# Unsigned-Long/slam-tricks

Hardware: AMD Instinct MI355X
Metric: LM iterations/sec + residuals/sec, 1k-cam/100k-pt BA (higher is better)
Workload: dtype f64

## Files before the change

include/stba.h:

```cpp
#ifndef STBA_H
#define STBA_H

#include <stddef.h>

#ifdef __cplusplus
extern "C" {
#endif

#define STBA_VERSION 6

enum {
    STBA_OK = 0,
    STBA_ERR_INVALID_ARGUMENT = -1,
    STBA_ERR_NO_DEVICE = -2,
    STBA_ERR_HIP = -3,
    STBA_ERR_NOT_POSITIVE_DEFINITE = -4,
    STBA_ERR_ALLOC = -5,
    STBA_ERR_STATE = -6,
    STBA_ERR_CALLBACK = -7,
    STBA_ERR_NO_SOLUTION = -8
};

const char* stba_status_string(int status);
const char* stba_last_error(void);
// ... 57 lines not shown
int stba_comm_create(stba_comm** out, const char id[STBA_COMM_ID_BYTES], int rank, int world_size, int device);
int stba_comm_destroy(stba_comm* comm);
int stba_comm_rank(const stba_comm* comm, int* rank, int* world_size);
int stba_comm_allreduce_sum(stba_comm* comm, void* buf_dev, size_t count, void* hip_stream);
int stba_comm_allreduce_hook(void* user, void* buf_dev, size_t count, void* hip_stream);

typedef struct stba_ba stba_ba;

int stba_ba_create(stba_ba** out, int n_cams, int n_pts, int n_obs, const double* cams,
                   const double* pts, const int* obs_cam, const int* obs_pt, const double* obs_feat,
                   const unsigned char* cam_fixed, const unsigned char* pt_fixed, void* hip_stream);
int stba_ba_destroy(stba_ba* ba);
enum { STBA_SCHUR_AUTO = 0, STBA_SCHUR_PAIRS = 1, STBA_SCHUR_DENSE = 2 };
int stba_ba_set_schur_mode(stba_ba* ba, int mode);
int stba_ba_schur_mode(const stba_ba* ba, int* mode);
int stba_ba_set_params(stba_ba* ba, const double* cams, const double* pts);
int stba_ba_get_params(stba_ba* ba, double* cams, double* pts);
int stba_ba_set_features(stba_ba* ba, const double* obs_feat);
int stba_get_device(int* device);
int stba_set_device(int device);
typedef int (*stba_ba_linearize_fn)(void* user, const double* cams, const double* pts, double* r, double* Jc, double* Jp);
int stba_ba_set_host_linearizer(stba_ba* ba, stba_ba_linearize_fn fn, void* user);
int stba_ba_set_allreduce(stba_ba* ba, stba_allreduce_fn fn, void* user, int rank, int world_size);
int stba_ba_set_comm(stba_ba* ba, stba_comm* comm);
int stba_ba_reduced_dim(const stba_ba* ba, int* n, int* n_padded);

int stba_ba_evaluate(stba_ba* ba, double* cost, double* r, double* Jc, double* Jp);
int stba_ba_cost(stba_ba* ba, double* cost);
int stba_ba_normal_blocks(stba_ba* ba, double* Hcc, double* gc, double* Hpp, double* gp);
int stba_ba_reduced_system(stba_ba* ba, const double* dc, const double* dp, double* S, double* rhs);
// ... 219 lines not shown
```

slam-tricks_amd/__init__.py:

```python
import ctypes as C
import os
import sys

import numpy as np

_HERE = os.path.dirname(os.path.abspath(__file__))
LIB_PATH = os.environ.get("STBA_LIB") or os.path.join(_HERE, "libstba.so")
TRACE_COLS = 7
TERM_REASON = {0: "none", 1: "gradient", 2: "function", 3: "parameter", 4: "max_iter",
               5: "min_radius", 6: "solver_fail", 7: "fixed", 8: "user"}
_lib = None


class StbaError(RuntimeError):
    def __init__(self, code, where):
        self.code = code
        msg = _lib.stba_last_error().decode() if _lib is not None else ""
        super().__init__(f"{where}: status {code} ({_lib.stba_status_string(code).decode()}) {msg}")


class LMOptions(C.Structure):
    _fields_ = [("max_num_iterations", C.c_int), ("initial_trust_region_radius", C.c_double),
                ("max_trust_region_radius", C.c_double), ("min_trust_region_radius", C.c_double),
                ("min_relative_decrease", C.c_double), ("min_lm_diagonal", C.c_double),
# ... 44 lines not shown
           "stba_ba_create_ex", "stba_ba_set_pcg", "stba_ba_last_pcg_summary", "stba_ba_schur_apply",
           "stba_ba_last_pcg_iterations", "stba_ba_time_schur_apply",
           "stba_ba_set_trust_region", "stba_ba_last_dogleg_summary",
           "stba_ba_set_inner_iterations", "stba_ba_inner_sweep", "stba_ba_last_inner_summary",
           "stba_pg_covariance_default_options", "stba_pg_covariance", "stba_pg_covariance_columns", "stba_pg_gauge_check",
           "stba_pg_set_information", "stba_pg_set_sqrt_information", "stba_pg_has_information",
           "stba_pg_set_loss", "stba_pg_has_loss",
           "stba_pg_set_priors", "stba_pg_prior_count", "stba_pg_evaluate_priors", "stba_pg_prior_kernel_geometry",
           "stba_ba_set_loss", "stba_ba_has_loss", "stba_ba_loss_kernel_geometry",
           "stba_ba_set_information", "stba_ba_set_sqrt_information", "stba_ba_has_information", "stba_ba_get_sqrt_information",
           "stba_ba_set_pose_priors", "stba_ba_pose_prior_count", "stba_ba_evaluate_pose_priors", "stba_ba_pose_prior_kernel_geometry",
           "stba_ba_set_relative_poses", "stba_ba_relative_pose_count", "stba_ba_evaluate_relative_poses",
           "stba_ba_relative_pose_kernel_geometry",
           "stba_ba_set_landmark_priors", "stba_ba_landmark_prior_count", "stba_ba_evaluate_landmark_priors",
           "stba_ba_landmark_prior_kernel_geometry",
           "stba_live_device_buffers"]


def lib():
    global _lib
    if _lib is None:
        if not os.path.exists(LIB_PATH):
            raise ImportError(f"{LIB_PATH} is missing: run `python __graft_entry__.py build` "
                              "(hipcc, gfx950).  There is no CPU fallback.")
        if "torch" not in sys.modules and os.environ.get("STBA_NO_TORCH_PRELOAD", "0") != "1":
            try:
                import torch
            except Exception:
                pass
        L = C.CDLL(LIB_PATH)
# ... 515 lines not shown
    def time_linearize(self, reps=20):
        ms = C.c_double()
        _chk(lib().stba_ba_time_linearize(self._h, int(reps), C.byref(ms)), "stba_ba_time_linearize")
        return ms.value

    SCHUR_AUTO, SCHUR_PAIRS, SCHUR_DENSE = 0, 1, 2

    def set_schur_mode(self, mode):
        _chk(lib().stba_ba_set_schur_mode(self._h, int(mode)), "stba_ba_set_schur_mode")

    def schur_mode(self):
        m = C.c_int()
        _chk(lib().stba_ba_schur_mode(self._h, C.byref(m)), "stba_ba_schur_mode")
        return m.value

    def set_pcg(self, preconditioner="jacobi", eta=0.1, min_iterations=0, max_iterations=500, check_every=4):
        pc = PRECONDITIONERS[preconditioner] if isinstance(preconditioner, str) else int(preconditioner)
        _chk(lib().stba_ba_set_pcg(self._h, pc, C.c_double(eta), int(min_iterations), int(max_iterations), int(check_every)),
             "stba_ba_set_pcg")

    def pcg_summary(self):
        s = PCGSummary()
        _chk(lib().stba_ba_last_pcg_summary(self._h, C.byref(s)), "stba_ba_last_pcg_summary")
        return s

    def pcg_iterations(self, n):
        out = np.zeros(int(n), dtype=np.int32)
        _chk(lib().stba_ba_last_pcg_iterations(self._h, _p(out), int(n)), "stba_ba_last_pcg_iterations")
        return out

# ... 506 lines not shown
```

slam-tricks_amd/build.py:

```python
import os
import subprocess
import sys

HERE = os.path.dirname(os.path.abspath(__file__))
CSRC = os.path.join(HERE, "csrc")
SOURCES = ["dense_chol.hip", "ba_kernels.hip", "stba_engine.hip", "ba_linear.hip", "ba_allreduce.hip", "ba_solve.hip", "ba_stages.hip", "dense_engine.hip", "calib.hip", "ba_factors.hip", "pg_engine.hip", "pg_linearize.hip", "pg_coarse.hip", "pg_pcg.hip", "pg_prior.hip", "small_dense.hip", "two_view.hip", "covariance.hip", "pg_covariance.hip", "iterative_schur.hip", "dogleg.hip", "inner_iterations.hip", "ba_prior.hip", "ba_between.hip", "ba_landmark_prior.hip", "calib_io.cpp", "comm.cpp"]
HEADERS = ["common.hpp", "lm_policy.hpp", "ba_kernels.hpp", "schur_plan.hpp", "chol_schedule.hpp", "small_linalg.hpp", "iterative_schur.hpp", "dogleg.hpp", "dogleg_select.hpp", "inner_iterations.hpp", "inner_policy.hpp", "pg_covariance.hpp", "robust_loss.hpp", "ba_prior.hpp", "ba_between.hpp", "ba_landmark_prior.hpp", "ba_features.hpp", "ba_factor_input.hpp", "ba_engine.hpp", "pg_plan.hpp", "pg_engine.hpp", "pg_device.hpp", "pg_edge.hpp", "inner_plan.hpp", "dd6.hpp", os.path.join("..", "..", "include", "stba.h")]
LIB = os.path.join(HERE, "libstba.so")
FLAGS = ["-O3", "-std=c++17", "--offload-arch=gfx950", "-fPIC", "-munsafe-fp-atomics", "-Wall",
         "-Wno-unused-function", "-Wno-unused-result"]


if os.environ.get("STBA_DEBUG_KNOBS", "0") not in ("", "0"):
    FLAGS.append("-DSTBA_DEBUG_KNOBS")


def _stale():
    if not os.path.exists(LIB):
        return True
    t = os.path.getmtime(LIB)
    deps = [os.path.join(CSRC, s) for s in SOURCES + HEADERS] + [os.path.abspath(__file__)]
    return any(os.path.getmtime(d) > t for d in deps)


# ... 63 lines not shown
```

slam-tricks_amd/csrc/ba_engine.hpp:

```cpp
#pragma once
#include <memory>
#include <vector>

#include "ba_kernels.hpp"
#include "ba_prior.hpp"
#include "ba_between.hpp"
#include "ba_landmark_prior.hpp"
#include "iterative_schur.hpp"
#include "ba_features.hpp"
#include "inner_plan.hpp"

namespace stba {

enum { SC_COST2 = 0, SC_GPMAX0 = 8, SC_MAX_WORLD = 64 };
enum { TS_COST2 = 0, TS_STEP2 = 1, TS_X2 = 2, TS_MODEL = 3, TS_TIMEOUT = 4, TS_CAM = 5, TS_COUNT = 8,
       TS_SPEC_COST2 = 8, TS_LIN_COST2 = 9, TS_LIN_GMAX = 10, TS_BLOCK = 11 };
enum { EV_LIN = 0, EV_LIN_END, EV_BUILD, EV_BUILD_END, EV_SOLVE_END, EV_BACKSUB_END, EV_TRIAL_END,
       EV_SPEC_A, EV_SPEC_A_END, EV_SPEC_B, EV_SPEC_B_END, EV_DBUILD, EV_DBUILD_END, EV_COUNT };

struct LossTable {
    DevBuf<int> kind;
    DevBuf<double> a, b, scale;
};

// ... 145 lines not shown
    DevBuf<double> Jc12;
    LossTable loss;
    DevBuf<double> winfo;
    DevBuf<unsigned char> omask;
    DevBuf<double> Hpp6, gp, Hinv6, Rinv9, dp, scale_p;
    DevBuf<double> Hcc, gc, cam_partial, dc, scale_c;
    DevBuf<double> Sbuf;
    DevBuf<double> dxc, dxp;
    DevBuf<double> cost_partial, upd_partial_c, upd_partial_p;
    DevBuf<double> trial;
    MappedBuffer ts_host;
    double ts_seq = 0.0;
    double ts_vals[TS_BLOCK] = {0};
    DevBuf<int> flag;
    int lin_grid = 1;
    CrossRankSum ar;
    bool have_lin = false, have_blocks = false, have_reduced = false, have_dxc = false, have_dxp = false;
    bool scale_init = false;
    DevEvent ev[EV_COUNT];
    CovStore* cov = nullptr;
    bool iterative = false;
    PcgSet pcg;
    DoglegSet dl;
    InnerSet inner;
    PriorSet prior;
    int lin_which = 0;
    BetweenSet btw;
    LandmarkPriorSet lprior;
    CostSlots cost_slots() const { return CostSlots{cost_partial, lin_grid, prior.n != 0, btw.n != 0, lprior.n != 0}; }
    int n_cost() const { return cost_slots().count(); }
// ... 20 lines not shown
    cov_store_free(b->cov);
    b->cov = nullptr;
}

inline int ba_factors_changed(stba_ba* b) {
    STBA_HIP(hipStreamSynchronize(b->st));
    ba_invalidate(b);
    ba_drop_covariance(b);
    return STBA_OK;
}

inline bool ba_wants_general_form(bool host_linearizer, bool loss, bool information) { return host_linearizer || loss || information; }
inline bool ba_wants_general_form(const stba_ba* b) { return ba_wants_general_form(b->hl.fn != nullptr, b->loss.kind.get() != nullptr, b->winfo.get() != nullptr); }
inline const double* ba_general_jc(const stba_ba* b) { return ba_wants_general_form(b) ? b->Jc12.get() : nullptr; }

inline int ba_refuse(const stba_ba* b, const char* who, bool sets = true) {
    const unsigned held = ba_held_features(b->iterative, b->dl.trust_region == STBA_TR_TRADITIONAL_DOGLEG, b->inner.on,b->hl.fn != nullptr,
                                           b->ar.fn != nullptr, b->loss.kind.get() != nullptr, b->winfo.get() != nullptr, b->prior.n, b->btw.n, b->lprior.n);
    std::string why;
    const int code = ba_conflict(who, held, &why, sets);
    return code ? fail(code, why) : STBA_OK;
}

#pragma GCC visibility push(hidden)

inline int refuse_iterative(const stba_ba* b, const char* who, const char* why) {
    if (!b || !b->iterative) return STBA_OK;
    return fail(STBA_ERR_INVALID_ARGUMENT, std::string(who) + ": this engine uses ITERATIVE_SCHUR, " + why);
}

int ba_linearize_dispatch(stba_ba* b, int which, bool with_jac);
int ba_linearize(stba_ba* b, int which, double* cost2_dev);
int ba_cost_only(stba_ba* b, int which, double* cost2_dev);
// ... 33 lines not shown
```

slam-tricks_amd/csrc/ba_features.hpp:

```cpp
#pragma once
#include <string>

#include "../../include/stba.h"

namespace stba {

enum BaFeature : unsigned {
    ITERATIVE_SCHUR = 1u << 0,
    DOGLEG = 1u << 1,
    INNER_ITERATIONS = 1u << 2,
    HOST_LINEARIZER = 1u << 3,
    ALLREDUCE = 1u << 4,
    LOSS = 1u << 5,
    INFORMATION = 1u << 6,
    POSE_PRIORS = 1u << 7,
    RELATIVE_POSES = 1u << 8,
    LANDMARK_PRIORS = 1u << 9
};
constexpr int BA_FEATURE_COUNT = 9;
constexpr int BA_FEATURE_COUNT_ALL = 10;

inline unsigned ba_held_features(bool iterative, bool dogleg, bool inner_on, bool host_linearizer, bool allreduce, bool loss,
                                 bool information, int n_priors, int n_relative_poses, int n_landmark_priors = 0) {
    return (iterative ? ITERATIVE_SCHUR : 0u) | (dogleg ? DOGLEG : 0u) | (inner_on ? INNER_ITERATIONS : 0u) |
           (host_linearizer ? HOST_LINEARIZER : 0u) | (allreduce ? ALLREDUCE : 0u) | (loss ? LOSS : 0u) |
           (information ? INFORMATION : 0u) | (n_priors ? POSE_PRIORS : 0u) | (n_relative_poses ? RELATIVE_POSES : 0u) |
           (n_landmark_priors ? LANDMARK_PRIORS : 0u);
}

struct BaRefusal {
    const char* asker;
    unsigned held;
    int code;
    const char* text;
    bool when_clearing = false;
};

#define STBA_INV STBA_ERR_INVALID_ARGUMENT
inline constexpr BaRefusal BA_REFUSALS[] = {
    {"stba_ba_set_host_linearizer", INNER_ITERATIONS, STBA_INV, "this engine has inner iterations (device residuals only)"},
    {"stba_ba_set_host_linearizer", LOSS, STBA_INV, "this engine has a loss table (losses need device residuals; not supported together)"},
    {"stba_ba_set_host_linearizer", INFORMATION, STBA_INV, "this engine has information matrices (the callback's factors whiten themselves; not supported together)"},
// ... 70 lines not shown
```

slam-tricks_amd/csrc/ba_kernels.hip:

```cpp
#include <algorithm>

#include "ba_kernels.hpp"
#include "robust_loss.hpp"
#include "small_linalg.hpp"

namespace stba {

template <bool CAMS_IN_LDS, bool WITH_JAC>
__global__ __launch_bounds__(LIN_THREADS) void ba_linearize_kernel(LinArgs a) {
    extern __shared__ __attribute__((aligned(16))) double smem[];
    double* s_j8 = smem;
    double* s_cam = smem + (WITH_JAC ? LIN_THREADS * 9 : 0);
    const int tid = threadIdx.x;
    if (CAMS_IN_LDS) {
        for (int i = tid; i < a.n_cams * 7; i += LIN_THREADS) s_cam[i] = a.cams[i];
        __syncthreads();
    }
    double cost = 0.0;
    const int n_tiles = (a.n_obs + LIN_THREADS - 1) / LIN_THREADS;
    for (int tile = blockIdx.x; tile < n_tiles; tile += gridDim.x) {
        const int base = tile * LIN_THREADS;
        const int i = base + tid;
        if (i < a.n_obs) {
            const double2 f = a.feat[i];
// ... 372 lines not shown
    double jc[12], jp[6];
    load_jc_jp<true>(J8, omask, i, jc, jp, Jc12);
    if (Jc) for (int k = 0; k < 12; ++k) Jc[(size_t)i * 12 + k] = jc[k];
    if (Jp) for (int k = 0; k < 6; ++k) Jp[(size_t)i * 6 + k] = jp[k];
}
int launch_expand_jacobian(int n_obs, const double* J8, const unsigned char* omask, double* Jc, double* Jp, hipStream_t st,
                           const double* Jc12) {
    if (n_obs > 0 && Jc12)
        hipLaunchKernelGGL(ba_expand_jacobian_gen_kernel, dim3((n_obs + 255) / 256), dim3(256), 0, st, n_obs, J8, omask, Jc12, Jc, Jp);
    else if (n_obs > 0) hipLaunchKernelGGL(ba_expand_jacobian_kernel, dim3((n_obs + 255) / 256), dim3(256), 0, st, n_obs, J8, omask, Jc, Jp);
    STBA_HIP(hipGetLastError());
    return STBA_OK;
}

constexpr int PB_LM = POINT_BLOCK_LANDMARKS, PB_THREADS = 128, PB_TRIPS = 2, PB_CHUNK = PB_TRIPS * PB_THREADS, PB_LD = PB_CHUNK + 1;
__global__ __launch_bounds__(PB_THREADS) void ba_point_blocks_kernel(int n_pts, const int* __restrict__ pt_start,
                                                                     const double* __restrict__ J8,
                                                                     const unsigned char* __restrict__ omask,
                                                                     const double2* __restrict__ r,
                                                                     double* __restrict__ Hpp6, double* __restrict__ gp,
                                                                     double* __restrict__ gpmax_partial) {
    __shared__ double u[9 * PB_LD];
    __shared__ int seg[PB_LM + 1];
    __shared__ double smax[PB_THREADS / 64];
    const int t = threadIdx.x;
    const int j0 = blockIdx.x * PB_LM, nl = min(PB_LM, n_pts - j0);
    if (t <= nl) seg[t] = pt_start[j0 + t];
    __syncthreads();
    const int rb = seg[0], re = seg[nl];
    double acc[3] = {0.0, 0.0, 0.0};
// ... 2 lines not shown
    lj[1] = (t + PB_THREADS) / 6; lk[1] = (t + PB_THREADS) % 6;
    lj[2] = t / 3; lk[2] = 6 + t % 3;
    if (t >= 3 * PB_LM) lj[2] = nl;
#pragma unroll
    for (int q = 0; q < 3; ++q) if (lj[q] > nl) lj[q] = nl;
    for (int cb = rb; cb < re; cb += PB_CHUNK) {
        const int ce = min(cb + PB_CHUNK, re);
#pragma unroll
        for (int s2 = 0; s2 < PB_TRIPS; ++s2) {
            const int x = t + PB_THREADS * s2, i = cb + x;
            if (i < ce) {
                const double2* p = reinterpret_cast<const double2*>(J8 + (size_t)i * 8);
                const double2 a = p[1], b = p[2], c = p[3];
                const double2 ri = r[i];
                const bool off = omask && (omask[i] & 64u);
                const double j00 = off ? 0.0 : a.x, j01 = off ? 0.0 : a.y, j02 = off ? 0.0 : b.x;
                const double j10 = off ? 0.0 : b.y, j11 = off ? 0.0 : c.x, j12 = off ? 0.0 : c.y;
                u[0 * PB_LD + x] = j00 * j00 + j10 * j10; u[1 * PB_LD + x] = j00 * j01 + j10 * j11; u[2 * PB_LD + x] = j00 * j02 + j10 * j12;
                u[3 * PB_LD + x] = j01 * j01 + j11 * j11; u[4 * PB_LD + x] = j01 * j02 + j11 * j12; u[5 * PB_LD + x] = j02 * j02 + j12 * j12;
                u[6 * PB_LD + x] = j00 * ri.x + j10 * ri.y; u[7 * PB_LD + x] = j01 * ri.x + j11 * ri.y; u[8 * PB_LD + x] = j02 * ri.x + j12 * ri.y;
            }
        }
        __syncthreads();
#pragma unroll
        for (int q = 0; q < 3; ++q) {
            if (lj[q] < nl) {
                const int b0 = max(seg[lj[q]], cb), e0 = min(seg[lj[q] + 1], ce);
                const double* uk = u + lk[q] * PB_LD - cb;
                for (int i = b0; i < e0; ++i) acc[q] += uk[i];
            }
        }
        __syncthreads();
    }
    if (lj[0] < nl) Hpp6[(size_t)j0 * 6 + t] = acc[0];
    if (lj[1] < nl) Hpp6[(size_t)j0 * 6 + t + PB_THREADS] = acc[1];
// ... 6 lines not shown
        if (t == 0) {
            double mm = 0.0;
            for (int w = 0; w < PB_THREADS / 64; ++w) mm = fmax(mm, smax[w]);
            gpmax_partial[blockIdx.x] = mm;
        }
    }
}

int point_blocks_grid(int n_pts) { return (n_pts + PB_LM - 1) / PB_LM; }

int launch_point_blocks(int n_pts, const int* pt_start, const double* J8, const unsigned char* omask, const double2* r,
                        double* Hpp6, double* gp, double* gpmax_partial, hipStream_t st) {
    if (n_pts > 0)
        hipLaunchKernelGGL(ba_point_blocks_kernel, dim3(point_blocks_grid(n_pts)), dim3(PB_THREADS), 0, st, n_pts, pt_start,
                           J8, omask, r, Hpp6, gp, gpmax_partial);
    STBA_HIP(hipGetLastError());
    return STBA_OK;
}

__global__ __launch_bounds__(256) void linear_finish_kernel(const double* __restrict__ cost_partial, int n_cost,
                                                            const double* __restrict__ gpmax_partial, int n_gp,
                                                            double* __restrict__ cost2_out, double* __restrict__ slots, int n_slots,
                                                            int cost_slot, int max_slot) {
    __shared__ double s[256], smx[256];
    double v = 0.0, m = 0.0;
#pragma unroll 4
    for (int i = threadIdx.x; i < n_cost; i += 256) v += cost_partial[i];
#pragma unroll 4
    for (int i = threadIdx.x; i < n_gp; i += 256) m = fmax(m, gpmax_partial[i]);
    s[threadIdx.x] = v;
// ... 1026 lines not shown
```

slam-tricks_amd/csrc/ba_kernels.hpp:

```cpp
#pragma once
#include "common.hpp"
#include "schur_plan.hpp"
#include "ba_landmark_prior.hpp"

namespace stba {

constexpr int LIN_THREADS = 1024;
constexpr int LIN_MAX_LDS = 160 * 1024 - 512;

struct LinArgs {
    int n_obs, n_cams;
    const double* cams;
    const double* pts;
    const double2* feat;
    const int* obs_cam;
    const int* obs_pt;
    const unsigned char* cam_fixed;
    const unsigned char* pt_fixed;
    double2* r;
    double* J8;
    double* cost_partial;
};

template <bool GEN = false>
// ... 24 lines not shown
    jc[7] = (m & 2u) ? 0.0 : -xn * yn;
    jc[8] = (m & 4u) ? 0.0 : -xn;
    const bool pf = (m & 64u) != 0u;
#pragma unroll
    for (int k = 0; k < 3; ++k) {
        const bool fx = (m >> (3 + k)) & 1u;
        jc[3 + k] = fx ? 0.0 : -P[k];
        jc[9 + k] = fx ? 0.0 : -P[3 + k];
        jp[k] = pf ? 0.0 : P[k];
        jp[3 + k] = pf ? 0.0 : P[3 + k];
    }
}

size_t lin_lds_bytes(int n_cams, bool cams_in_lds, bool with_jac);
int launch_linearize(const LinArgs& a, bool with_jac, int grid, hipStream_t st);
constexpr int LIN_ROBUST_THREADS = 512;
struct LinLoss {
    const int* kind;
    const double* a;
    const double* b;
    const double* scale;
    double* Jc12;
    const double* winfo;
};
size_t lin_robust_lds_bytes(int n_cams, bool cams_in_lds, bool with_jac);
bool lin_robust_cams_in_lds(int n_cams);
int launch_linearize_robust(const LinArgs& a, const LinLoss& l, bool with_jac, int grid, hipStream_t st);
int launch_sum_partials(const double* partial, int n, int stride, int K, double* out, hipStream_t st);
int launch_expand_jacobian(int n_obs, const double* J8, const unsigned char* omask, double* Jc, double* Jp, hipStream_t st,
                           const double* Jc12 = nullptr);
// ... 117 lines not shown
```

slam-tricks_amd/csrc/ba_linear.hip:

```cpp
#include <algorithm>
#include <vector>

#include "ba_engine.hpp"

namespace stba {

static LinArgs lin_args(stba_ba* b, int which, bool store_r) {
    LinArgs a;
    a.n_obs = b->no; a.n_cams = b->nc;
    a.cams = b->cams[which]; a.pts = b->pts[which];
    a.feat = b->feat; a.obs_cam = b->obs_cam; a.obs_pt = b->obs_pt;
    a.cam_fixed = b->cam_fixed; a.pt_fixed = b->pt_fixed;
    a.r = store_r ? b->r : nullptr; a.J8 = b->J8; a.cost_partial = b->cost_partial;
    return a;
}

static int ba_host_linearize(stba_ba* b, int which, bool with_jac) {
    const size_t no = (size_t)b->no;
    b->hl.cams.resize((size_t)b->nc * 7); b->hl.pts.resize((size_t)b->np * 3); b->hl.r.resize(no * 2);
    if (with_jac) { b->hl.jc.resize(no * 12); b->hl.jp.resize(no * 6); }
    STBA_TRY(download(b->hl.cams.data(), b->cams[which], b->hl.cams.size(), b->st));
    STBA_TRY(download(b->hl.pts.data(), b->pts[which], b->hl.pts.size(), b->st));
    STBA_HIP(hipStreamSynchronize(b->st));
    if (b->hl.fn(b->hl.user, b->hl.cams.data(), b->hl.pts.data(), b->hl.r.data(), with_jac ? b->hl.jc.data() : nullptr,
// ... 15 lines not shown
        for (size_t p = 0; p < no; ++p) {
            const size_t i = (size_t)b->perm[p];
            st[p * 8] = 0.0; st[p * 8 + 1] = 0.0;
            memcpy(&st[p * 8 + 2], &b->hl.jp[i * 6], 6 * sizeof(double));
        }
        STBA_TRY(upload(b->J8, st.data(), no * 8, b->st));
        STBA_HIP(hipStreamSynchronize(b->st));
        for (size_t p = 0; p < no; ++p) memcpy(&st[p * 12], &b->hl.jc[(size_t)b->perm[p] * 12], 12 * sizeof(double));
        STBA_TRY(upload(b->Jc12, st.data(), no * 12, b->st));
        STBA_HIP(hipStreamSynchronize(b->st));
    }
    return STBA_OK;
}

int ba_linearize_dispatch(stba_ba* b, int which, bool with_jac) {
    if (b->hl.fn) return ba_host_linearize(b, which, with_jac);
    const LinArgs a = lin_args(b, which, with_jac);
    if (with_jac) b->lin_which = which;
    if (b->loss.kind || b->winfo)
        STBA_TRY(launch_linearize_robust(a, LinLoss{b->loss.kind, b->loss.a, b->loss.b, b->loss.scale, b->Jc12, b->winfo}, with_jac, b->lin_grid, b->st));
    else
        STBA_TRY(launch_linearize(a, with_jac, b->lin_grid, b->st));
    const CostSlots slots = b->cost_slots();
    if (b->prior.n) STBA_TRY(launch_prior_cost(b->prior_args(), b->cams[which], slots.pose_priors(), b->st));
    if (b->btw.n) STBA_TRY(launch_between_cost(b->between_args(), b->cams[which], slots.relative_poses(), b->st));
    if (b->lprior.n) STBA_TRY(launch_landmark_prior_cost(b->landmark_prior_args(), b->pts[which], b->lprior.cost_part, slots.landmark_priors(), b->st));
    return STBA_OK;
}

int ba_prior_blocks(stba_ba* b) {
    if (!b->prior.n) return STBA_OK;
    return launch_prior_blocks(b->prior_args(), b->cams[b->lin_which], b->Hcc, b->gc, nullptr, nullptr, b->st);
}

int ba_between_blocks(stba_ba* b, bool with_S) {
// ... 1 lines not shown
    return launch_between_blocks(b->between_args(), b->cams[b->lin_which], b->Hcc, b->gc, with_S ? b->S() : nullptr, b->lda, nullptr, nullptr,
                                 nullptr, b->st);
}

int ba_linearize(stba_ba* b, int which, double* cost2_dev) {
    STBA_TRY(ba_linearize_dispatch(b, which, true));
    return launch_sum_partials(b->cost_partial, b->n_cost(), 1, 1, cost2_dev, b->st);
}

int ba_cost_only(stba_ba* b, int which, double* cost2_dev) {
    STBA_TRY(ba_linearize_dispatch(b, which, false));
    return launch_sum_partials(b->cost_partial, b->n_cost(), 1, 1, cost2_dev, b->st);
}

int ba_normal_blocks(stba_ba* b) {
    STBA_TRY(launch_point_blocks(b->np, b->pt_start, b->J8, b->omask, b->r, b->Hpp6, b->gp, b->upd_partial_p, b->st));
    if (!b->lprior.n) return STBA_OK;
    return launch_landmark_prior_blocks(b->landmark_prior_args(), b->pts[b->lin_which], b->Hpp6, b->gp, b->upd_partial_p, nullptr, nullptr, b->st);
}
int ba_linearize_lm(stba_ba* b, int which) {
    return ba_linearize_dispatch(b, which, true);
}
int ba_camera_blocks(stba_ba* b) {
    return launch_camera_blocks(b->nc, b->n_chunks, b->chunk_begin, b->chunk_end, b->cam_chunk_start, b->cam_perm,
                                b->J8, b->omask, ba_general_jc(b), b->r, b->cam_partial, b->Hcc, b->gc, b->st);
}

int ba_dense_alloc(stba_ba* b) {
    if (b->schur.Y) return STBA_OK;
    const size_t kcols = ((size_t)3 * b->np + 15) / 16 * 16;
// ... 66 lines not shown
    if (!dm.explicit_d && b->n == 6 * b->nc) {
        STBA_TRY(launch_reduced_finalize(b->nc, b->n, b->Hcc, b->gc, b->cam_fixed, b->S(), b->lda, b->rhs(), b->ex_diag(), b->ex_gc(),
                                         b->scale_c, init_scale, dm.use_scaling, dm.radius, dm.dmin, dm.dmax, b->dc, 1, b->st));
        b->scale_init = true;
        return STBA_OK;
    }
    if (!dm.explicit_d)
        STBA_TRY(launch_lm_diagonal(b->n, 1, 1, 2, b->ex_diag(), b->scale_c, init_scale, dm.use_scaling, dm.radius,
                                    dm.dmin, dm.dmax, b->dc, b->st));
    b->scale_init = true;
    STBA_TRY(launch_reduced_damp(b->n, b->dc, b->cam_fixed, b->S(), b->lda, b->rhs(), b->st));
    return chol_prepare_padding_dev(b->S(), b->lda, b->n, b->rhs(), b->st);
}

int ba_fill_scalar_slots(stba_ba* b, double* cost2_dev) {
    return launch_linear_finish(b->cost_partial, b->n_cost(), b->upd_partial_p, point_blocks_grid(b->np), cost2_dev, b->ex_scalar(), b->lda,
                                SC_COST2, SC_GPMAX0 + b->ar.rank, b->st);
}

__global__ void export_trial_kernel(const double* __restrict__ trial, const int* __restrict__ flag, double* __restrict__ out, double seq) {
    __shared__ double hp[TS_BLOCK];
    const int k = threadIdx.x;
    if (k == TS_SPEC_COST2) hp[k] = (double)flag[0];
    else if (k < TS_BLOCK) hp[k] = trial[k];
    __syncthreads();
    stamped_store_wave(out, hp, TS_BLOCK, seq, k);
}

int ba_backsub_trial(stba_ba* b) {
    BacksubUpdate up{b->pts[b->cur], b->pt_fixed, b->dp, b->pts[b->cur ^ 1], b->upd_partial_p,
                     b->nc, b->cams[b->cur], b->cam_fixed, b->ex_gc(), b->dc, b->cams[b->cur ^ 1], b->upd_partial_c};
// ... 156 lines not shown
```

slam-tricks_amd/csrc/stba_engine.hip:

```cpp
#include <algorithm>
#include <chrono>
#include <memory>
#include <vector>

#include "ba_engine.hpp"
#include "inner_iterations.hpp"
#include "lm_policy.hpp"

namespace stba {

thread_local std::string g_last_error;

int require_device() {
    int n = 0;
    hipError_t e = hipGetDeviceCount(&n);
    if (e != hipSuccess || n <= 0)
        return fail(STBA_ERR_NO_DEVICE, std::string("no HIP device visible (") +
                                            (e == hipSuccess ? "count=0" : hipGetErrorString(e)) +
                                            "); libstba has no CPU fallback");
    return STBA_OK;
}

}

// ... 95 lines not shown
    b->schur.plan_mode = P.plan_mode;
    b->schur.pairs = (double)P.pairs; b->schur.lds_atomics = P.lds_atomics;
    std::vector<unsigned char> cmask;
    if (cam_fixed) {
        cmask.resize(n_cams);
        for (int c = 0; c < n_cams; ++c) {
            unsigned m = 0;
            for (int a = 0; a < 6; ++a) if (cam_fixed[c * 6 + a]) m |= (1u << a);
            cmask[c] = (unsigned char)m;
        }
    }
    const int n_tiles = (n_obs + LIN_THREADS - 1) / LIN_THREADS;
    const size_t lds = lin_lds_bytes(n_cams, lin_lds_bytes(n_cams, true, true) <= (size_t)LIN_MAX_LDS, true);
    const int per_cu = std::max(1, std::min(4, (int)((160 * 1024) / std::max<size_t>(lds, 1))));
    b->lin_grid = std::max(1, std::min(n_tiles, num_cu * per_cu));

    tmark("masks");
    const size_t no = (size_t)n_obs, np = (size_t)n_pts, nc = (size_t)n_cams;
    const std::string who = "stba_ba_create";
    STBA_TRY(to_device(who, b->cams[0], cams, nc * 7, b->st)); STBA_TRY(to_device(who, b->pts[0], pts, np * 3, b->st));
    STBA_TRY(b->cams[1].alloc(nc * 7)); STBA_TRY(b->pts[1].alloc(np * 3));
    STBA_TRY(b->feat.alloc(no));
    STBA_TRY(upload(reinterpret_cast<double*>(b->feat.get()), P.s_feat.data(), no * 2, b->st));
    STBA_TRY(to_device(who, b->obs_cam, P.s_cam, b->st)); STBA_TRY(to_device(who, b->obs_pt, P.s_pt, b->st));
    STBA_TRY(to_device(who, b->pt_start, P.pt_start, b->st)); STBA_TRY(to_device(who, b->cam_perm, P.cam_perm, b->st));
    STBA_TRY(to_device(who, b->chunk_begin, P.chunk_begin, b->st)); STBA_TRY(to_device(who, b->chunk_end, P.chunk_end, b->st));
    STBA_TRY(to_device(who, b->cam_chunk_start, P.cam_chunk_start, b->st));
    STBA_TRY(to_device(who, b->schur.task_cam, P.task_cam, b->st)); STBA_TRY(to_device(who, b->schur.cam_start, P.cam_start, b->st));
    STBA_TRY(to_device(who, b->schur.task_col_lo, P.task_col_lo, b->st)); STBA_TRY(to_device(who, b->schur.task_col_hi, P.task_col_hi, b->st));
    b->ar.h_row_col_ptr = P.row_col_ptr; b->ar.h_row_cols = P.row_cols;
    STBA_TRY(to_device(who, b->schur.row_col_ptr, P.row_col_ptr, b->st)); STBA_TRY(to_device(who, b->schur.row_cols, P.row_cols, b->st));
    STBA_TRY(to_device(who, b->schur.pair_begin, P.pair_begin, b->st)); STBA_TRY(to_device(who, b->schur.pair_end, P.pair_end, b->st));
    STBA_TRY(b->schur.pair_rec.alloc(P.pairs));
    if (P.pairs > 0) STBA_TRY(upload(b->schur.pair_rec, reinterpret_cast<const int4*>(P.pair_rec.get()), P.pairs, b->st));
    STBA_TRY(to_device(who, b->schur.task_vs_ptr, P.task_vs_ptr, b->st)); STBA_TRY(to_device(who, b->schur.vs_first, P.vs_first, b->st));
    if (cam_fixed) STBA_TRY(to_device(who, b->cam_fixed, cmask, b->st));
    if (pt_fixed) STBA_TRY(to_device(who, b->pt_fixed, pt_fixed, np, b->st));
    if (b->schur.lm_slices) {
        STBA_TRY(to_device(who, b->schur.task_p_lo, P.task_p_lo, b->st)); STBA_TRY(to_device(who, b->schur.task_p_hi, P.task_p_hi, b->st));
        STBA_TRY(to_device(who, b->schur.task_part_off, P.task_part_off, b->st));
        STBA_TRY(to_device(who, b->schur.row_task_ptr, P.row_task_ptr, b->st)); STBA_TRY(to_device(who, b->schur.row_tasks, P.row_tasks, b->st));
        STBA_TRY(b->schur.part.alloc(P.part_doubles));
// ... 1 lines not shown
    if (!P.dup_run.empty()) STBA_TRY(to_device(who, b->schur.dup_run, P.dup_run, b->st));
    std::vector<unsigned char>& omask = b->schur.create_omask;
    if (cam_fixed || pt_fixed) {
        omask.resize(no);
        for (size_t p2 = 0; p2 < no; ++p2)
            omask[p2] = (unsigned char)((cam_fixed ? cmask[(size_t)P.s_cam[p2]] : 0u) | ((pt_fixed && pt_fixed[(size_t)P.s_pt[p2]]) ? 64u : 0u));
        STBA_TRY(to_device(who, b->omask, omask, b->st));
    }
    STBA_TRY(b->r.alloc(no)); STBA_TRY(b->J8.alloc(no * 8));
    STBA_TRY(b->Hpp6.alloc(np * 6)); STBA_TRY(b->gp.alloc(np * 3)); STBA_TRY(b->Hinv6.alloc(np * 6)); STBA_TRY(b->Rinv9.alloc(np * 9));
    STBA_TRY(b->dp.alloc(np * 3)); STBA_TRY(b->scale_p.alloc(np * 3));
    STBA_TRY(b->Hcc.alloc(nc * 36)); STBA_TRY(b->gc.alloc(nc * 6)); STBA_TRY(b->cam_partial.alloc((size_t)b->n_chunks * 28));
    STBA_TRY(b->dc.alloc(nc * 6)); STBA_TRY(b->scale_c.alloc(nc * 6));
    STBA_TRY(b->Sbuf.alloc(b->sbuf_count()));
    STBA_TRY(b->dxc.alloc((size_t)b->lda)); STBA_TRY(b->dxp.alloc(np * 3));
    STBA_TRY(b->cost_partial.alloc(CostSlots::capacity(b->lin_grid)));
    STBA_TRY(b->upd_partial_c.alloc((size_t)backsub_cam_grid(n_cams) * 4));
    STBA_TRY(b->upd_partial_p.alloc((size_t)(point_blocks_grid(n_pts) + 1) * 4));
    STBA_TRY(b->trial.alloc((size_t)TS_BLOCK)); STBA_TRY(b->flag.alloc(1));
    if (iterative) STBA_TRY(ba_pcg_alloc(b));

    if (hipMemsetAsync(b->dxc, 0, (size_t)b->lda * sizeof(double), b->st) != hipSuccess ||
        hipMemsetAsync(b->Sbuf, 0, b->sbuf_count() * sizeof(double), b->st) != hipSuccess ||
        hipStreamSynchronize(b->st) != hipSuccess)
        return fail(STBA_ERR_HIP, "stba_ba_create: initial memset/sync failed");
    tmark("device arrays, uploads + sync");
    b->perm = std::move(plan->perm);
    b->schur.create_leftovers = std::move(plan);
    return STBA_OK;
}

// ... 72 lines not shown
    STBA_TRY(refuse_iterative(ba, "stba_ba_set_schur_mode", "which forms no Schur complement"));
    if (!ba || mode < STBA_SCHUR_AUTO || mode > STBA_SCHUR_DENSE) return fail(STBA_ERR_INVALID_ARGUMENT, "stba_ba_set_schur_mode: bad argument");
    if (mode == STBA_SCHUR_AUTO) mode = ba->schur.mode_auto;
    if (mode == STBA_SCHUR_PAIRS && !ba->schur.have_pair_plan)
        return fail(STBA_ERR_INVALID_ARGUMENT, "stba_ba_set_schur_mode: this engine was created without a pair plan (too many observation pairs)");
    if (mode == STBA_SCHUR_DENSE && ba->schur.dup_overflow)
        return fail(STBA_ERR_INVALID_ARGUMENT, "stba_ba_set_schur_mode: more than 255 observations of one (camera, landmark) pair: the dense form cannot take this problem");
    if (mode == STBA_SCHUR_DENSE) STBA_TRY(ba_dense_alloc(ba));
    ba->schur.mode = mode;
    ba->have_reduced = ba->have_dxc = ba->have_dxp = false;
    return STBA_OK;
}
int stba_ba_schur_mode(const stba_ba* ba, int* mode) {
    if (!ba || !mode) return fail(STBA_ERR_INVALID_ARGUMENT, "stba_ba_schur_mode: bad argument");
    *mode = ba->schur.mode;
    return STBA_OK;
}

int stba_ba_destroy(stba_ba* ba) {
    if (!ba) return STBA_OK;
    ba_free(ba);
    return STBA_OK;
}

int stba_ba_set_params(stba_ba* b, const double* cams, const double* pts) {
    if (!b) return fail(STBA_ERR_INVALID_ARGUMENT, "null engine");
    if (cams) STBA_TRY(upload(b->cams[b->cur], cams, (size_t)b->nc * 7, b->st));
    if (pts) STBA_TRY(upload(b->pts[b->cur], pts, (size_t)b->np * 3, b->st));
    STBA_HIP(hipStreamSynchronize(b->st));
    ba_invalidate(b);
// ... 133 lines not shown
```

Baseline: 371.0.

## Fuse landmark Hpp/gp block accumulation into the Jacobian linearize kernel

Adds a linearize kernel that computes residuals and J8, and in the same pass builds the per-landmark 3x3 Hessian blocks and gradients from values still in registers and LDS. Observations that spill past a tile boundary are recomputed in a bounded tail. This removes the separate point-blocks launch and its re-read of J8 and residuals, at the cost of redundant tail recomputation, more LDS per block and extra syncthreads. It is used by default when no loss, information, host linearizer or landmark priors are set and the longest tail fits.

```diff
diff --git a/include/stba.h b/include/stba.h
--- a/include/stba.h
+++ b/include/stba.h
@@ -95,6 +95,9 @@
 enum { STBA_SCHUR_AUTO = 0, STBA_SCHUR_PAIRS = 1, STBA_SCHUR_DENSE = 2 };
 int stba_ba_set_schur_mode(stba_ba* ba, int mode);
 int stba_ba_schur_mode(const stba_ba* ba, int* mode);
+enum { STBA_LANDMARK_BLOCKS_AUTO = 0, STBA_LANDMARK_BLOCKS_SEPARATE = 1 };
+int stba_ba_set_landmark_blocks(stba_ba* ba, int mode);
+int stba_ba_landmark_blocks_geometry(const stba_ba* ba, int* in_jacobian_kernel, int* tile_observations, int* longest_tail, int* tail_capacity);
 int stba_ba_set_params(stba_ba* ba, const double* cams, const double* pts);
 int stba_ba_get_params(stba_ba* ba, double* cams, double* pts);
 int stba_ba_set_features(stba_ba* ba, const double* obs_feat);
diff --git a/slam-tricks_amd/__init__.py b/slam-tricks_amd/__init__.py
--- a/slam-tricks_amd/__init__.py
+++ b/slam-tricks_amd/__init__.py
@@ -82,6 +82,7 @@
            "stba_ba_relative_pose_kernel_geometry",
            "stba_ba_set_landmark_priors", "stba_ba_landmark_prior_count", "stba_ba_evaluate_landmark_priors",
            "stba_ba_landmark_prior_kernel_geometry",
+           "stba_ba_set_landmark_blocks", "stba_ba_landmark_blocks_geometry",
            "stba_live_device_buffers"]
 
 
@@ -627,6 +628,16 @@
         _chk(lib().stba_ba_schur_mode(self._h, C.byref(m)), "stba_ba_schur_mode")
         return m.value
 
+    LANDMARK_BLOCKS_AUTO, LANDMARK_BLOCKS_SEPARATE = 0, 1
+
+    def set_landmark_blocks(self, mode):
+        _chk(lib().stba_ba_set_landmark_blocks(self._h, int(mode)), "stba_ba_set_landmark_blocks")
+
+    def landmark_blocks_geometry(self):
+        f, t, m, c = C.c_int(), C.c_int(), C.c_int(), C.c_int()
+        _chk(lib().stba_ba_landmark_blocks_geometry(self._h, C.byref(f), C.byref(t), C.byref(m), C.byref(c)), "stba_ba_landmark_blocks_geometry")
+        return bool(f.value), t.value, m.value, c.value
+
     def set_pcg(self, preconditioner="jacobi", eta=0.1, min_iterations=0, max_iterations=500, check_every=4):
         pc = PRECONDITIONERS[preconditioner] if isinstance(preconditioner, str) else int(preconditioner)
         _chk(lib().stba_ba_set_pcg(self._h, pc, C.c_double(eta), int(min_iterations), int(max_iterations), int(check_every)),
diff --git a/slam-tricks_amd/build.py b/slam-tricks_amd/build.py
--- a/slam-tricks_amd/build.py
+++ b/slam-tricks_amd/build.py
@@ -5,7 +5,7 @@
 HERE = os.path.dirname(os.path.abspath(__file__))
 CSRC = os.path.join(HERE, "csrc")
 SOURCES = ["dense_chol.hip", "ba_kernels.hip", "stba_engine.hip", "ba_linear.hip", "ba_allreduce.hip", "ba_solve.hip", "ba_stages.hip", "dense_engine.hip", "calib.hip", "ba_factors.hip", "pg_engine.hip", "pg_linearize.hip", "pg_coarse.hip", "pg_pcg.hip", "pg_prior.hip", "small_dense.hip", "two_view.hip", "covariance.hip", "pg_covariance.hip", "iterative_schur.hip", "dogleg.hip", "inner_iterations.hip", "ba_prior.hip", "ba_between.hip", "ba_landmark_prior.hip", "calib_io.cpp", "comm.cpp"]
-HEADERS = ["common.hpp", "lm_policy.hpp", "ba_kernels.hpp", "schur_plan.hpp", "chol_schedule.hpp", "small_linalg.hpp", "iterative_schur.hpp", "dogleg.hpp", "dogleg_select.hpp", "inner_iterations.hpp", "inner_policy.hpp", "pg_covariance.hpp", "robust_loss.hpp", "ba_prior.hpp", "ba_between.hpp", "ba_landmark_prior.hpp", "ba_features.hpp", "ba_factor_input.hpp", "ba_engine.hpp", "pg_plan.hpp", "pg_engine.hpp", "pg_device.hpp", "pg_edge.hpp", "inner_plan.hpp", "dd6.hpp", os.path.join("..", "..", "include", "stba.h")]
+HEADERS = ["common.hpp", "lm_policy.hpp", "ba_kernels.hpp", "schur_plan.hpp", "lin_tiles.hpp", "chol_schedule.hpp", "small_linalg.hpp", "iterative_schur.hpp", "dogleg.hpp", "dogleg_select.hpp", "inner_iterations.hpp", "inner_policy.hpp", "pg_covariance.hpp", "robust_loss.hpp", "ba_prior.hpp", "ba_between.hpp", "ba_landmark_prior.hpp", "ba_features.hpp", "ba_factor_input.hpp", "ba_engine.hpp", "pg_plan.hpp", "pg_engine.hpp", "pg_device.hpp", "pg_edge.hpp", "inner_plan.hpp", "dd6.hpp", os.path.join("..", "..", "include", "stba.h")]
 LIB = os.path.join(HERE, "libstba.so")
 FLAGS = ["-O3", "-std=c++17", "--offload-arch=gfx950", "-fPIC", "-munsafe-fp-atomics", "-Wall",
          "-Wno-unused-function", "-Wno-unused-result"]
diff --git a/slam-tricks_amd/csrc/ba_engine.hpp b/slam-tricks_amd/csrc/ba_engine.hpp
--- a/slam-tricks_amd/csrc/ba_engine.hpp
+++ b/slam-tricks_amd/csrc/ba_engine.hpp
@@ -183,6 +183,10 @@
     double ts_vals[TS_BLOCK] = {0};
     DevBuf<int> flag;
     int lin_grid = 1;
+    DevBuf<int> lin_tile_lm;
+    DevBuf<double> lin_gpmax;
+    int lin_max_tail = 0;
+    bool lin_blocks_separate = false, lin_made_blocks = false;
     CrossRankSum ar;
     bool have_lin = false, have_blocks = false, have_reduced = false, have_dxc = false, have_dxp = false;
     bool scale_init = false;
@@ -233,9 +237,16 @@
 inline bool ba_wants_general_form(const stba_ba* b) { return ba_wants_general_form(b->hl.fn != nullptr, b->loss.kind.get() != nullptr, b->winfo.get() != nullptr); }
 inline const double* ba_general_jc(const stba_ba* b) { return ba_wants_general_form(b) ? b->Jc12.get() : nullptr; }
 
+inline unsigned ba_held(const stba_ba* b) {
+    return ba_held_features(b->iterative, b->dl.trust_region == STBA_TR_TRADITIONAL_DOGLEG, b->inner.on,b->hl.fn != nullptr,
+                            b->ar.fn != nullptr, b->loss.kind.get() != nullptr, b->winfo.get() != nullptr, b->prior.n, b->btw.n, b->lprior.n);
+}
+inline bool ba_blocks_in_linearize(const stba_ba* b) {
+    return ba_blocks_in_linearize(ba_held(b), lin_blocks_fit(b->nc, b->no, b->lin_max_tail), b->lin_blocks_separate);
+}
+
 inline int ba_refuse(const stba_ba* b, const char* who, bool sets = true) {
-    const unsigned held = ba_held_features(b->iterative, b->dl.trust_region == STBA_TR_TRADITIONAL_DOGLEG, b->inner.on,b->hl.fn != nullptr,
-                                           b->ar.fn != nullptr, b->loss.kind.get() != nullptr, b->winfo.get() != nullptr, b->prior.n, b->btw.n, b->lprior.n);
+    const unsigned held = ba_held(b);
     std::string why;
     const int code = ba_conflict(who, held, &why, sets);
     return code ? fail(code, why) : STBA_OK;
diff --git a/slam-tricks_amd/csrc/ba_features.hpp b/slam-tricks_amd/csrc/ba_features.hpp
--- a/slam-tricks_amd/csrc/ba_features.hpp
+++ b/slam-tricks_amd/csrc/ba_features.hpp
@@ -26,6 +26,10 @@
            (host_linearizer ? HOST_LINEARIZER : 0u) | (allreduce ? ALLREDUCE : 0u) | (loss ? LOSS : 0u) |
            (information ? INFORMATION : 0u) | (n_priors ? POSE_PRIORS : 0u) | (n_relative_poses ? RELATIVE_POSES : 0u) |
            (n_landmark_priors ? LANDMARK_PRIORS : 0u);
+}
+
+inline bool ba_blocks_in_linearize(unsigned held, bool fits, bool separate) {
+    return fits && !separate && !(held & (HOST_LINEARIZER | LOSS | INFORMATION | LANDMARK_PRIORS));
 }
 
 struct BaRefusal {
diff --git a/slam-tricks_amd/csrc/ba_kernels.hip b/slam-tricks_amd/csrc/ba_kernels.hip
--- a/slam-tricks_amd/csrc/ba_kernels.hip
+++ b/slam-tricks_amd/csrc/ba_kernels.hip
@@ -410,6 +410,14 @@
 }
 
 constexpr int PB_LM = POINT_BLOCK_LANDMARKS, PB_THREADS = 128, PB_TRIPS = 2, PB_CHUNK = PB_TRIPS * PB_THREADS, PB_LD = PB_CHUNK + 1;
+__device__ __forceinline__ void point_block_products(double p00, double p01, double p02, double p10, double p11, double p12,
+                                                     double2 ri, bool off, double* __restrict__ u, int ld) {
+    const double j00 = off ? 0.0 : p00, j01 = off ? 0.0 : p01, j02 = off ? 0.0 : p02;
+    const double j10 = off ? 0.0 : p10, j11 = off ? 0.0 : p11, j12 = off ? 0.0 : p12;
+    u[0 * ld] = j00 * j00 + j10 * j10; u[1 * ld] = j00 * j01 + j10 * j11; u[2 * ld] = j00 * j02 + j10 * j12;
+    u[3 * ld] = j01 * j01 + j11 * j11; u[4 * ld] = j01 * j02 + j11 * j12; u[5 * ld] = j02 * j02 + j12 * j12;
+    u[6 * ld] = j00 * ri.x + j10 * ri.y; u[7 * ld] = j01 * ri.x + j11 * ri.y; u[8 * ld] = j02 * ri.x + j12 * ri.y;
+}
 __global__ __launch_bounds__(PB_THREADS) void ba_point_blocks_kernel(int n_pts, const int* __restrict__ pt_start,
                                                                      const double* __restrict__ J8,
                                                                      const unsigned char* __restrict__ omask,
@@ -442,11 +450,7 @@
                 const double2 a = p[1], b = p[2], c = p[3];
                 const double2 ri = r[i];
                 const bool off = omask && (omask[i] & 64u);
-                const double j00 = off ? 0.0 : a.x, j01 = off ? 0.0 : a.y, j02 = off ? 0.0 : b.x;
-                const double j10 = off ? 0.0 : b.y, j11 = off ? 0.0 : c.x, j12 = off ? 0.0 : c.y;
-                u[0 * PB_LD + x] = j00 * j00 + j10 * j10; u[1 * PB_LD + x] = j00 * j01 + j10 * j11; u[2 * PB_LD + x] = j00 * j02 + j10 * j12;
-                u[3 * PB_LD + x] = j01 * j01 + j11 * j11; u[4 * PB_LD + x] = j01 * j02 + j11 * j12; u[5 * PB_LD + x] = j02 * j02 + j12 * j12;
-                u[6 * PB_LD + x] = j00 * ri.x + j10 * ri.y; u[7 * PB_LD + x] = j01 * ri.x + j11 * ri.y; u[8 * PB_LD + x] = j02 * ri.x + j12 * ri.y;
+                point_block_products(a.x, a.y, b.x, b.y, c.x, c.y, ri, off, u + x, PB_LD);
             }
         }
         __syncthreads();
@@ -483,6 +487,116 @@
     if (n_pts > 0)
         hipLaunchKernelGGL(ba_point_blocks_kernel, dim3(point_blocks_grid(n_pts)), dim3(PB_THREADS), 0, st, n_pts, pt_start,
                            J8, omask, r, Hpp6, gp, gpmax_partial);
+    STBA_HIP(hipGetLastError());
+    return STBA_OK;
+}
+
+constexpr int LB_LD = LIN_THREADS + LIN_TAIL + 1;
+__device__ __forceinline__ void lin_observation(const double* cam, const double* L, double2 f, double& r0, double& r1, double& xn,
+                                                double& yn, double P[6]) {
+    double q[4] = {cam[0], cam[1], cam[2], cam[3]};
+    const double t0 = cam[4], t1 = cam[5], t2 = cam[6];
+    const double d0 = L[0] - t0, d1 = L[1] - t1, d2 = L[2] - t2;
+    double R[9];
+    quat_to_rot(q, R);
+    const double x = R[0] * d0 + R[3] * d1 + R[6] * d2;
+    const double y = R[1] * d0 + R[4] * d1 + R[7] * d2;
+    const double z = R[2] * d0 + R[5] * d1 + R[8] * d2;
+    const double iz = 1.0 / z;
+    xn = x * iz; yn = y * iz;
+    r0 = xn - f.x; r1 = yn - f.y;
+#pragma unroll
+    for (int k = 0; k < 3; ++k) {
+        P[k] = iz * (R[k * 3 + 0] - xn * R[k * 3 + 2]);
+        P[3 + k] = iz * (R[k * 3 + 1] - yn * R[k * 3 + 2]);
+    }
+}
+
+__global__ __launch_bounds__(LIN_THREADS) void ba_linearize_blocks_kernel(LinArgs a, LinBlocks lb) {
+    extern __shared__ __attribute__((aligned(16))) double smem[];
+    double* s_j8 = smem;
+    double* s_cam = smem + 9 * LB_LD;
+    const int tid = threadIdx.x;
+    for (int i = tid; i < a.n_cams * 7; i += LIN_THREADS) s_cam[i] = a.cams[i];
+    __syncthreads();
+    double cost = 0.0, gmax = 0.0;
+    const int n_tiles = (a.n_obs + LIN_THREADS - 1) / LIN_THREADS;
+    for (int tile = blockIdx.x; tile < n_tiles; tile += gridDim.x) {
+        const int base = tile * LIN_THREADS;
+        const int i = base + tid;
+        double P[6] = {0.0, 0.0, 0.0, 0.0, 0.0, 0.0};
+        double2 ri = make_double2(0.0, 0.0);
+        if (i < a.n_obs) {
+            double xn, yn;
+            lin_observation(s_cam + a.obs_cam[i] * 7, a.pts + (size_t)a.obs_pt[i] * 3, a.feat[i], ri.x, ri.y, xn, yn, P);
+            a.r[i] = ri;
+            cost += ri.x * ri.x + ri.y * ri.y;
+            double* j8 = s_j8 + tid * 9;
+            j8[0] = xn; j8[1] = yn;
+#pragma unroll
+            for (int k = 0; k < 6; ++k) j8[2 + k] = P[k];
+        }
+        __syncthreads();
+        const int n_here = min(LIN_THREADS, a.n_obs - base);
+        double* gj = a.J8 + (size_t)base * 8;
+        for (int e = tid; e < n_here * 4; e += LIN_THREADS) {
+            const int o = e >> 2, k = (e & 3) * 2;
+            const double* sj = s_j8 + o * 9 + k;
+            *reinterpret_cast<double2*>(gj + 2 * (size_t)e) = make_double2(sj[0], sj[1]);
+        }
+        __syncthreads();
+        const int l0 = lb.tile_lm[tile], l1 = lb.tile_lm[tile + 1], nl = l1 - l0;
+        const int tail = nl > 0 ? min(max(lb.pt_start[l1] - (base + LIN_THREADS), 0), LIN_TAIL) : 0;
+        if (i < a.n_obs) point_block_products(P[0], P[1], P[2], P[3], P[4], P[5], ri, lb.omask && (lb.omask[i] & 64u), s_j8 + tid, LB_LD);
+        if (tid < tail) {
+            const int it = base + LIN_THREADS + tid;
+            double xn, yn, Pt[6];
+            double2 rt;
+            lin_observation(s_cam + a.obs_cam[it] * 7, a.pts + (size_t)a.obs_pt[it] * 3, a.feat[it], rt.x, rt.y, xn, yn, Pt);
+            point_block_products(Pt[0], Pt[1], Pt[2], Pt[3], Pt[4], Pt[5], rt, lb.omask && (lb.omask[it] & 64u), s_j8 + LIN_THREADS + tid, LB_LD);
+        }
+        __syncthreads();
+        for (int e = tid; e < nl * 9; e += LIN_THREADS) {
+            const bool g = e >= nl * 6;
+            const int e2 = g ? e - nl * 6 : e, j = l0 + (g ? e2 / 3 : e2 / 6), k = g ? 6 + e2 % 3 : e2 % 6;
+            const int b0 = lb.pt_start[j] - base, e0 = lb.pt_start[j + 1] - base;
+            const double* uk = s_j8 + k * LB_LD;
+            double acc = 0.0;
+            for (int x = b0; x < e0; ++x) acc += uk[x];
+            if (g) { lb.gp[(size_t)l0 * 3 + e2] = acc; gmax = fmax(gmax, fabs(acc)); }
+            else lb.Hpp6[(size_t)l0 * 6 + e2] = acc;
+        }
+        __syncthreads();
+    }
+    __shared__ double s_red[LIN_THREADS / 64], s_max[LIN_THREADS / 64];
+    for (int off = 32; off > 0; off >>= 1) {
+        cost += __shfl_down(cost, off, 64);
+        gmax = fmax(gmax, __shfl_down(gmax, off, 64));
+    }
+    if ((tid & 63) == 0) { s_red[tid >> 6] = cost; s_max[tid >> 6] = gmax; }
+    __syncthreads();
+    if (tid == 0) {
+        double s = 0.0, m = 0.0;
+        for (int w = 0; w < LIN_THREADS / 64; ++w) { s += s_red[w]; m = fmax(m, s_max[w]); }
+        a.cost_partial[blockIdx.x] = s;
+        lb.gpmax_partial[blockIdx.x] = m;
+    }
+}
+
+size_t lin_blocks_lds_bytes(int n_cams) { return ((size_t)9 * LB_LD + (size_t)n_cams * 7) * sizeof(double) + 16; }
+
+bool lin_blocks_fit(int n_cams, int n_obs, int max_tail) {
+    return n_obs > 0 && max_tail <= LIN_TAIL && lin_blocks_lds_bytes(n_cams) <= (size_t)LIN_MAX_LDS;
+}
+
+int launch_linearize_blocks(const LinArgs& a, const LinBlocks& lb, int grid, hipStream_t st) {
+    static DeviceOnce attr;
+    STBA_TRY(attr.run([]() -> int {
+        STBA_HIP(hipFuncSetAttribute(reinterpret_cast<const void*>(ba_linearize_blocks_kernel), hipFuncAttributeMaxDynamicSharedMemorySize,
+                                     LIN_MAX_LDS));
+        return STBA_OK;
+    }));
+    hipLaunchKernelGGL(ba_linearize_blocks_kernel, dim3(grid), dim3(LIN_THREADS), lin_blocks_lds_bytes(a.n_cams), st, a, lb);
     STBA_HIP(hipGetLastError());
     return STBA_OK;
 }
diff --git a/slam-tricks_amd/csrc/ba_kernels.hpp b/slam-tricks_amd/csrc/ba_kernels.hpp
--- a/slam-tricks_amd/csrc/ba_kernels.hpp
+++ b/slam-tricks_amd/csrc/ba_kernels.hpp
@@ -1,6 +1,7 @@
 #pragma once
 #include "common.hpp"
 #include "schur_plan.hpp"
+#include "lin_tiles.hpp"
 #include "ba_landmark_prior.hpp"
 
 namespace stba {
@@ -62,6 +63,16 @@
 
 size_t lin_lds_bytes(int n_cams, bool cams_in_lds, bool with_jac);
 int launch_linearize(const LinArgs& a, bool with_jac, int grid, hipStream_t st);
+struct LinBlocks {
+    const int* tile_lm;
+    const int* pt_start;
+    const unsigned char* omask;
+    double* Hpp6; double* gp;
+    double* gpmax_partial;
+};
+size_t lin_blocks_lds_bytes(int n_cams);
+bool lin_blocks_fit(int n_cams, int n_obs, int max_tail);
+int launch_linearize_blocks(const LinArgs& a, const LinBlocks& lb, int grid, hipStream_t st);
 constexpr int LIN_ROBUST_THREADS = 512;
 struct LinLoss {
     const int* kind;
diff --git a/slam-tricks_amd/csrc/ba_linear.hip b/slam-tricks_amd/csrc/ba_linear.hip
--- a/slam-tricks_amd/csrc/ba_linear.hip
+++ b/slam-tricks_amd/csrc/ba_linear.hip
@@ -53,11 +53,14 @@
 }
 
 int ba_linearize_dispatch(stba_ba* b, int which, bool with_jac) {
+    if (with_jac) b->lin_made_blocks = ba_blocks_in_linearize(b);
     if (b->hl.fn) return ba_host_linearize(b, which, with_jac);
     const LinArgs a = lin_args(b, which, with_jac);
     if (with_jac) b->lin_which = which;
     if (b->loss.kind || b->winfo)
         STBA_TRY(launch_linearize_robust(a, LinLoss{b->loss.kind, b->loss.a, b->loss.b, b->loss.scale, b->Jc12, b->winfo}, with_jac, b->lin_grid, b->st));
+    else if (with_jac && b->lin_made_blocks)
+        STBA_TRY(launch_linearize_blocks(a, LinBlocks{b->lin_tile_lm, b->pt_start, b->omask, b->Hpp6, b->gp, b->lin_gpmax}, b->lin_grid, b->st));
     else
         STBA_TRY(launch_linearize(a, with_jac, b->lin_grid, b->st));
     const CostSlots slots = b->cost_slots();
@@ -89,6 +92,7 @@
 }
 
 int ba_normal_blocks(stba_ba* b) {
+    if (b->lin_made_blocks) return STBA_OK;
     STBA_TRY(launch_point_blocks(b->np, b->pt_start, b->J8, b->omask, b->r, b->Hpp6, b->gp, b->upd_partial_p, b->st));
     if (!b->lprior.n) return STBA_OK;
     return launch_landmark_prior_blocks(b->landmark_prior_args(), b->pts[b->lin_which], b->Hpp6, b->gp, b->upd_partial_p, nullptr, nullptr, b->st);
@@ -185,7 +189,9 @@
 }
 
 int ba_fill_scalar_slots(stba_ba* b, double* cost2_dev) {
-    return launch_linear_finish(b->cost_partial, b->n_cost(), b->upd_partial_p, point_blocks_grid(b->np), cost2_dev, b->ex_scalar(), b->lda,
+    const double* gpmax = b->lin_made_blocks ? b->lin_gpmax.get() : b->upd_partial_p.get();
+    const int n_gpmax = b->lin_made_blocks ? b->lin_grid : point_blocks_grid(b->np);
+    return launch_linear_finish(b->cost_partial, b->n_cost(), gpmax, n_gpmax, cost2_dev, b->ex_scalar(), b->lda,
                                 SC_COST2, SC_GPMAX0 + b->ar.rank, b->st);
 }
 
diff --git a/slam-tricks_amd/csrc/lin_tiles.hpp b/slam-tricks_amd/csrc/lin_tiles.hpp
--- /dev/null
+++ b/slam-tricks_amd/csrc/lin_tiles.hpp
@@ -0,0 +1,29 @@
+#pragma once
+#include <algorithm>
+#include <vector>
+
+namespace stba {
+
+constexpr int LIN_TAIL = 128;
+
+struct LinTiles {
+    std::vector<int> tile_lm;
+    int max_tail = 0;
+};
+
+inline LinTiles build_lin_tiles(int n_obs, int n_pts, const int* pt_start, int tile) {
+    LinTiles t;
+    const int n_tiles = (n_obs + tile - 1) / tile;
+    t.tile_lm.resize((size_t)n_tiles + 1);
+    for (int k = 0; k < n_tiles; ++k)
+        t.tile_lm[(size_t)k] = (int)(std::lower_bound(pt_start, pt_start + n_pts, (int)std::min<long long>((long long)k * tile, n_obs)) - pt_start);
+    t.tile_lm[(size_t)n_tiles] = n_pts;
+    for (int k = 0; k < n_tiles; ++k) {
+        const long long tile_end = std::min<long long>((long long)(k + 1) * tile, n_obs);
+        if (t.tile_lm[(size_t)k + 1] > t.tile_lm[(size_t)k])
+            t.max_tail = std::max<long long>(t.max_tail, pt_start[t.tile_lm[(size_t)k + 1]] - tile_end);
+    }
+    return t;
+}
+
+}
diff --git a/slam-tricks_amd/csrc/stba_engine.hip b/slam-tricks_amd/csrc/stba_engine.hip
--- a/slam-tricks_amd/csrc/stba_engine.hip
+++ b/slam-tricks_amd/csrc/stba_engine.hip
@@ -133,6 +133,9 @@
     const size_t lds = lin_lds_bytes(n_cams, lin_lds_bytes(n_cams, true, true) <= (size_t)LIN_MAX_LDS, true);
     const int per_cu = std::max(1, std::min(4, (int)((160 * 1024) / std::max<size_t>(lds, 1))));
     b->lin_grid = std::max(1, std::min(n_tiles, num_cu * per_cu));
+    const LinTiles tiles = build_lin_tiles(n_obs, n_pts, P.pt_start.data(), LIN_THREADS);
+    b->lin_max_tail = tiles.max_tail;
+    if (knob_int("STBA_LIN_BLOCKS_SEPARATE", 0) != 0) b->lin_blocks_separate = true;
 
     tmark("masks");
     const size_t no = (size_t)n_obs, np = (size_t)n_pts, nc = (size_t)n_cams;
@@ -145,6 +148,7 @@
     STBA_TRY(to_device(who, b->pt_start, P.pt_start, b->st)); STBA_TRY(to_device(who, b->cam_perm, P.cam_perm, b->st));
     STBA_TRY(to_device(who, b->chunk_begin, P.chunk_begin, b->st)); STBA_TRY(to_device(who, b->chunk_end, P.chunk_end, b->st));
     STBA_TRY(to_device(who, b->cam_chunk_start, P.cam_chunk_start, b->st));
+    STBA_TRY(to_device(who, b->lin_tile_lm, tiles.tile_lm, b->st));
     STBA_TRY(to_device(who, b->schur.task_cam, P.task_cam, b->st)); STBA_TRY(to_device(who, b->schur.cam_start, P.cam_start, b->st));
     STBA_TRY(to_device(who, b->schur.task_col_lo, P.task_col_lo, b->st)); STBA_TRY(to_device(who, b->schur.task_col_hi, P.task_col_hi, b->st));
     b->ar.h_row_col_ptr = P.row_col_ptr; b->ar.h_row_cols = P.row_cols;
@@ -176,7 +180,7 @@
     STBA_TRY(b->dc.alloc(nc * 6)); STBA_TRY(b->scale_c.alloc(nc * 6));
     STBA_TRY(b->Sbuf.alloc(b->sbuf_count()));
     STBA_TRY(b->dxc.alloc((size_t)b->lda)); STBA_TRY(b->dxp.alloc(np * 3));
-    STBA_TRY(b->cost_partial.alloc(CostSlots::capacity(b->lin_grid)));
+    STBA_TRY(b->cost_partial.alloc(CostSlots::capacity(b->lin_grid))); STBA_TRY(b->lin_gpmax.alloc((size_t)b->lin_grid));
     STBA_TRY(b->upd_partial_c.alloc((size_t)backsub_cam_grid(n_cams) * 4));
     STBA_TRY(b->upd_partial_p.alloc((size_t)(point_blocks_grid(n_pts) + 1) * 4));
     STBA_TRY(b->trial.alloc((size_t)TS_BLOCK)); STBA_TRY(b->flag.alloc(1));
@@ -279,6 +283,22 @@
 int stba_ba_schur_mode(const stba_ba* ba, int* mode) {
     if (!ba || !mode) return fail(STBA_ERR_INVALID_ARGUMENT, "stba_ba_schur_mode: bad argument");
     *mode = ba->schur.mode;
+    return STBA_OK;
+}
+
+int stba_ba_set_landmark_blocks(stba_ba* ba, int mode) {
+    if (!ba || (mode != STBA_LANDMARK_BLOCKS_AUTO && mode != STBA_LANDMARK_BLOCKS_SEPARATE))
+        return fail(STBA_ERR_INVALID_ARGUMENT, "stba_ba_set_landmark_blocks: bad argument");
+    ba->lin_blocks_separate = mode == STBA_LANDMARK_BLOCKS_SEPARATE;
+    ba_invalidate(ba);
+    return STBA_OK;
+}
+int stba_ba_landmark_blocks_geometry(const stba_ba* ba, int* in_jacobian_kernel, int* tile_observations, int* longest_tail, int* tail_capacity) {
+    if (!ba) return fail(STBA_ERR_INVALID_ARGUMENT, "stba_ba_landmark_blocks_geometry: null engine");
+    if (in_jacobian_kernel) *in_jacobian_kernel = ba_blocks_in_linearize(ba) ? 1 : 0;
+    if (tile_observations) *tile_observations = LIN_THREADS;
+    if (longest_tail) *longest_tail = ba->lin_max_tail;
+    if (tail_capacity) *tail_capacity = LIN_TAIL;
     return STBA_OK;
 }
 
```

Result: no change. 371.8 (median of 2 runs) (+0.2%).
